# BMCV/SuperDSM

Hardware: AMD Instinct MI355X
Metric: candidate DSM solves/sec (higher is better)
Workload: dtype f64; 1 GPU; bbbc039_like 520x696 (BASELINE.json configs[1] stand-in: ellipses at the centres/areas of 8 different reference BBBC039 regression tables), 8 images per step in ONE launch, all candidates of every image: connected atom subsets of size <= 3 + cluster universes; gather_payload_bytes_per_rank=0, ranks=1, ranks_per_gpu=1, devices_visible=1, median_N=1325, median_M=23, parallelism=single GPU, steps_in_flight=1

## Files before the change

include/sdsm.h:

```cpp
#ifndef SDSM_H
#define SDSM_H

#include <stddef.h>
#include <stdint.h>

#ifdef __cplusplus
extern "C" {
#endif

#define SDSM_VERSION 200

typedef enum {
    SDSM_OK = 0,
    SDSM_ERR_ARGUMENT = -1,
    SDSM_ERR_DEVICE = -2,
    SDSM_ERR_WORKSPACE = -3,
    SDSM_ERR_UNSUPPORTED = -4
} sdsm_status;

typedef struct {
    double scale;
    double epsilon;
    double alpha;
    double smooth_amount;
// ... 61 lines not shown
size_t sdsm_plan_workspace_bytes(const sdsm_plan *plan);
size_t sdsm_plan_mask_bytes(const sdsm_plan *plan);
int sdsm_plan_describe(const sdsm_plan *plan, int32_t *mask_info, int64_t *mask_offset, int32_t *n_pixels);
int64_t sdsm_plan_total_pixels(const sdsm_plan *plan);

int sdsm_batch_upload(const sdsm_plan *plan, void *d_workspace, size_t workspace_bytes, void *stream);
int sdsm_batch_launch(const sdsm_plan *plan, const double *d_y, const int32_t *d_atoms, const uint8_t *d_valid,
                      void *d_workspace, size_t workspace_bytes, sdsm_record *d_records, uint32_t *d_masks,
                      double *d_xi, void *stream);
int sdsm_batch_launch_multi(const sdsm_plan *plan, const double *const *d_y, const int32_t *const *d_atoms, const uint8_t *const *d_valid,
                            void *d_workspace, size_t workspace_bytes, sdsm_record *d_records, uint32_t *d_masks, double *d_xi, void *stream);
int64_t sdsm_plan_xi_count(const sdsm_plan *plan);
int sdsm_plan_layout(const sdsm_plan *plan, int64_t *out);
int sdsm_plan_set_latency_mode(sdsm_plan *plan, int mode);
int sdsm_plan_schedule(const sdsm_plan *plan, int32_t *group_members, int32_t *rows_workgroups);
int sdsm_plan_xi_offsets(const sdsm_plan *plan, int64_t *xi_offset);

typedef struct {
    double contrast;
    double interior_mean;
    double exterior_mean;
    double fg_mean, fg_std;
    int32_t area;
    int32_t status;
    int32_t r0, c0, h, w;
} sdsm_post_record;
int sdsm_post_objects(const double *d_g, const double *d_gs, const uint8_t *d_bg, int H, int W, int n, const int32_t *d_boxes,
                      const int64_t *d_bits_off, const uint32_t *d_bits, const int64_t *d_new_off, uint32_t *d_new_bits,
                      uint32_t *d_boundary_pool, const int64_t *d_bpool_off, double exterior_scale, double exterior_offset,
                      double contrast_epsilon, double inv_gstd, int max_distance, double stdamp, sdsm_post_record *d_out, void *stream);
// ... 218 lines not shown
```

superdsm_amd/_capi.py:

```python
import ctypes as C
import os

import numpy as np

_HERE = os.path.dirname(os.path.abspath(__file__))
LIB_PATH = os.environ.get('SDSM_HIP_LIB', os.path.join(_HERE, 'libsdsm_hip.so'))

SDSM_OK = 0
ATOM_STATS_STRIDE = 6

CAND_OPTIMAL, CAND_FALLBACK, CAND_TRIVIAL, CAND_ERROR, CAND_UNSUPPORTED, CAND_GIVEN_UP = 0, 1, 2, 3, 4, 5


class DsmConfig(C.Structure):
    _fields_ = [('scale', C.c_double), ('epsilon', C.c_double), ('alpha', C.c_double), ('smooth_amount', C.c_double),
                ('gaussian_shape_multiplier', C.c_double), ('background_margin', C.c_double),
                ('smooth_subsample', C.c_int32), ('init_elliptical', C.c_int32), ('max_iters', C.c_int32), ('flags', C.c_int32)]


RECORD_DTYPE = np.dtype([
    ('energy', 'f8'), ('theta', 'f8', 6), ('energy_ell', 'f8'),
    ('status', 'i4'), ('flags', 'i4'), ('n_pixels', 'i4'), ('n_deform', 'i4'),
    ('iters_ell', 'i4'), ('iters_dsm', 'i4'), ('evals_value', 'i4'), ('evals_full', 'i4'),
    ('on_boundary', 'i4'), ('fg_r0', 'i4'), ('fg_c0', 'i4'), ('fg_h', 'i4'), ('fg_w', 'i4'), ('n_positive', 'i4'), ('n_negative', 'i4'), ('reserved', 'i4')])
# ... 63 lines not shown
    'sdsm_image_prepare': (_i32, [_vp, _vp, _vp, _i32, _i32, _f64, _i32, _vp, _vp, _vp, _sz, _vp]),
    'sdsm_plan_create': (_vp, [_i32, _i32, _i32, _vp, C.POINTER(DsmConfig), _i32, _vp, _vp]),
    'sdsm_plan_create_multi': (_vp, [_i32, _vp, _vp, _vp, _vp, C.POINTER(DsmConfig), _i32, _vp, _vp, _vp]),
    'sdsm_plan_destroy': (None, [_vp]),
    'sdsm_plan_workspace_bytes': (_sz, [_vp]),
    'sdsm_plan_mask_bytes': (_sz, [_vp]),
    'sdsm_plan_describe': (_i32, [_vp, _vp, _vp, _vp]),
    'sdsm_plan_total_pixels': (_i64, [_vp]),
    'sdsm_batch_upload': (_i32, [_vp, _vp, _sz, _vp]),
    'sdsm_batch_launch': (_i32, [_vp, _vp, _vp, _vp, _vp, _sz, _vp, _vp, _vp, _vp]),
    'sdsm_batch_launch_multi': (_i32, [_vp, _vp, _vp, _vp, _vp, _sz, _vp, _vp, _vp, _vp]),
    'sdsm_plan_xi_count': (_i64, [_vp]),
    'sdsm_plan_xi_offsets': (_i32, [_vp, _vp]),
    'sdsm_plan_layout': (_i32, [_vp, _vp]),
    'sdsm_plan_schedule': (_i32, [_vp, _vp, _vp]),
    'sdsm_plan_set_latency_mode': (_i32, [_vp, _i32]),
    'sdsm_post_objects': (_i32, [_vp, _vp, _vp, _i32, _i32, _i32, _vp, _vp, _vp, _vp, _vp, _vp, _vp, _f64, _f64, _f64, _f64, _i32, _f64, _vp, _vp]),
    'sdsm_post_objects_multi': (_i32, [C.POINTER(PostImage), _i32, _vp, _vp, _vp, _vp, _vp, _vp, _vp, _f64, _f64, _f64, _i32, _f64, _vp, _vp]),
    'sdsm_post_background_multi': (_i32, [C.POINTER(PostBgImage), _i32, _vp, _vp, _vp, _i32, _vp]),
    'sdsm_post_fill_holes': (_i32, [_i32, _vp, _vp, _vp, _vp, _vp, _vp, _vp, _vp]),
    'sdsm_post_glare_multi': (_i32, [C.POINTER(PostImage), _i32, _vp, _vp, _vp, C.POINTER(C.c_double), _i32, _vp, _vp, _vp, _vp]),
    'sdsm_gaussian_workspace_bytes': (_sz, [_i32, _i32, _f64]),
    'sdsm_gaussian_filter': (_i32, [_vp, _i32, _i32, _f64, _vp, _vp, _sz, _vp]),
    'sdsm_separable_workspace_bytes': (_sz, [_i32, _i32, _i32, _i32]),
    'sdsm_separable_filter': (_i32, [_vp, _i32, _i32, _vp, _i32, _vp, _i32, _vp, _vp, _sz, _vp]),
    'sdsm_log_masks_workspace_bytes': (_sz, [_i32, _i32]),
    'sdsm_log_masks': (_i32, [_vp, _i32, _i32, _i32, _vp, _vp, _vp, _vp, _sz, _vp]),
    'sdsm_integral_image': (_i32, [_vp, _i32, _i32, _vp, _vp]),
    'sdsm_doh_cube': (_i32, [_vp, _i32, _i32, _i32, _vp, _vp, _vp, _vp, _vp]),
    'sdsm_doh_peaks': (_i32, [_vp, _i32, _i32, _i32, _f64, _vp, _i64, _vp]),
# ... 103 lines not shown
```

superdsm_amd/csrc/sdsm_api.hip:

```cpp
#include <algorithm>
#include <atomic>
#include <cmath>
#include <cstdio>
#include <cstdlib>
#include <cstring>
#include <numeric>
#include <string>
#include <vector>

#include "sdsm_common.h"
#include <climits>

extern "C" hipError_t sdsm_launch_solve(const BatchParams &P, sdsm_record *records, uint32_t *masks, double *xi_out, hipStream_t stream,
                                        hipStream_t side1, hipStream_t side2, hipStream_t side3, hipStream_t side4, hipEvent_t *ev, int n_c, int n_d, int n_w, int n_r);
extern "C" hipError_t sdsm_image_prepare_impl(const double *, const uint8_t *, const int32_t *, int, int, double, int, uint8_t *, int32_t *, void *, hipStream_t);
extern "C" hipError_t sdsm_preprocess_impl(const double *, int, int, double, double, double, int, double *, void *, hipStream_t);
extern "C" void sdsm_gauss_kernel_host(double sigma, int radius, double *w);
extern "C" hipError_t sdsm_launch_setup(const BatchParams &P, hipStream_t stream, const int32_t *order_w, int n_w, int cls, const int32_t *order_small, int n_small, const int32_t *order_big, int n_big);
extern "C" int sdsm_setup_fits_small(int h, int w, int mcap, int max_label, int k);
extern "C" int sdsm_setup_class(int max_dim, int max_mcap, int max_label, int k);

static thread_local std::string g_err;
static int fail(int code, const std::string &msg) { g_err = msg; return code; }
static int hipfail(hipError_t e, const char *what) { return fail(SDSM_ERR_DEVICE, std::string(what) + ": " + hipGetErrorString(e)); }
// ... 96 lines not shown
struct sdsm_plan {
    int n = 0;
    std::vector<PlanImage> images;
    sdsm_dsm_config cfg{};
    int k = 1, R = 0, zcap = 1, zcap_run = 1, zshift = 0, no_deform = 0;
    std::vector<CandDesc> cand;
    std::vector<int32_t> fp_labels, order;
    int n_order_c = 0, n_order_d = 0, n_order_w = 0;
    int n_order_r = 0;
    int rows_mcap = 1;
    int n_setup_small = 0, n_setup_big = 0, max_label = 1;
    int setup_class = 2;
    int mode = 0;
    int wide_pixels = INT_MAX;
    int boost_pixels = INT_MAX;
    std::vector<float> psf;
    std::vector<int32_t> mask_info, n_pixels;
    std::vector<int64_t> mask_off_bytes, xi_off;
    int64_t total_pixels = 0, total_runs = 0, total_ell = 0, total_xi = 0, total_mask_words = 0, n_hglob = 0, n_wide = 0;
    size_t off_cand = 0, off_state = 0, off_fp = 0, off_order = 0, off_crop_y = 0, off_crop_rc = 0, off_crop_cc = 0, off_dist = 0, off_tmp_y = 0, off_tmp_rc = 0, off_inv = 0, off_run_meta = 0,
           off_run_q0 = 0, off_run_aux = 0, off_grid = 0, off_ell_im = 0, off_ell_w = 0, off_psf = 0, off_env_fst = 0, off_env_rb = 0, off_hglob = 0, off_wide = 0, off_ticket = 0, total = 0;
    uint64_t layout_gen = 0;
    mutable const double *x0 = nullptr;
    mutable uint64_t uploaded_gen = 0;
    mutable const void *uploaded_ws = nullptr;
    mutable SideSet *sides = nullptr;
};

#include <mutex>
static std::mutex g_pool_mutex;
static std::vector<SideSet *> g_side_sets;

static hipError_t acquire_sides(const sdsm_plan *p, hipStream_t caller)
{
    int dev = 0;
    hipError_t e = hipGetDevice(&dev);
    if (e != hipSuccess) return e;
    int sdev = dev;
    if (caller && hipStreamGetDevice(caller, &sdev) == hipSuccess && sdev != dev) return hipErrorInvalidDevice;
    (void)hipGetLastError();
    if (p->sides) return p->sides->device == dev ? hipSuccess : hipErrorInvalidDevice;
    std::lock_guard<std::mutex> lock(g_pool_mutex);
    for (SideSet *q : g_side_sets) if (q->device == dev) { p->sides = q; return hipSuccess; }
    SideSet *s = new SideSet();
    s->device = dev;
// ... 27 lines not shown
#ifndef SDSM_ROWS_MAX_REGIONS
#define SDSM_ROWS_MAX_REGIONS 1024
#endif
#ifndef SDSM_WIDE_TP_MIN_PIXELS
#define SDSM_WIDE_TP_MIN_PIXELS 8192
#endif
#ifndef SDSM_K1_PIXDIV
#define SDSM_K1_PIXDIV 2048
#endif
#ifndef SDSM_WIDE_FILL
#define SDSM_WIDE_FILL 1024
#endif
#ifndef SDSM_WIDE_MAX_MEMBERS
#define SDSM_WIDE_MAX_MEMBERS 256
#endif
static void layout_plan(sdsm_plan *p)
{
    const int n = p->n;
    const bool latency = p->mode == 1, groups = p->mode != 2;
    p->wide_pixels = latency ? SDSM_WIDE_PIXELS : INT_MAX;
    p->boost_pixels = INT_MAX;
    p->layout_gen++;
    p->n_wide = 0;
    long long wide_thr = SDSM_WIDE_MIN_PIXELS;
    if (groups && !latency) {
        long long all_pixels = 0;
        for (int i = 0; i < n; i++) all_pixels += p->cand[i].N;
        long long tp_min = SDSM_WIDE_TP_MIN_PIXELS;
        if (const char *e = getenv("SDSM_WIDE_TP_MIN_PIXELS")) { const long long v = atoll(e); if (v > 0) tp_min = v; }
        wide_thr = std::max<long long>(tp_min, all_pixels / SDSM_WIDE_FILL);
// ... 1 lines not shown
    if (!latency) {
        long long all_pixels = 0;
        for (int i = 0; i < n; i++) all_pixels += p->cand[i].N;
        long long div = SDSM_K1_PIXDIV;
        if (const char *e = getenv("SDSM_K1_PIXDIV")) { const long long v = atoll(e); if (v > 0) div = v; else if (v < 0) div = 0; }
        p->boost_pixels = div > 0 ? (int)std::min<long long>(INT_MAX, std::max<long long>(SDSM_WIDE_PIXELS, all_pixels / div)) : INT_MAX;
    }
    long wide_slice = SDSM_WIDE_SLICE;
    if (const char *e = getenv("SDSM_WIDE_SLICE")) { const long v = atol(e); if (v > 0) wide_slice = v; }
    auto group_size = [&](long N) -> long {
        if (!groups || n >= (1 << 24)) return 0;
        if (N > wide_thr) return std::min<long>(SDSM_WIDE_MAX_G, std::max<long>(2, (N + wide_slice - 1) / wide_slice));
        if (latency && N > SDSM_WIDE_PIXELS) return std::min<long>(SDSM_LAT_GMAX, std::max<long>(2, (N + SDSM_LAT_SLICE - 1) / SDSM_LAT_SLICE));
        return 0;
    };
    std::vector<char> grouped(n, 1);
    {
        std::vector<int> big;
        for (int i = 0; i < n; i++) if (group_size(p->cand[i].N) > 0) big.push_back(i);
        std::stable_sort(big.begin(), big.end(), [&](int a, int b) { return p->cand[a].N > p->cand[b].N; });
        long members = 0;
        int cutoff = 0;
        for (int i : big) {
            members += group_size(p->cand[i].N);
            if (members > SDSM_WIDE_MAX_MEMBERS) { cutoff = p->cand[i].N; break; }
        }
        for (int i : big) if (p->cand[i].N <= cutoff) grouped[i] = 0;
    }
    long rows_regions = 0;
    for (int i = 0; i < n; i++) rows_regions += p->cand[i].N > SDSM_ROWS_MIN_PIXELS;
    const bool rows_multi = rows_regions <= SDSM_ROWS_MAX_REGIONS;
    for (int i = 0; i < n; i++) {
        CandDesc &c = p->cand[i];
        const long G = grouped[i] ? group_size(c.N) : 0;
        const long RG = rows_multi && c.N > SDSM_ROWS_MIN_PIXELS && n < (1 << 24) ? std::min<long>(SDSM_ROWS_MAX_G, (c.N + SDSM_ROWS_SLICE - 1) / SDSM_ROWS_SLICE) : 0;
        c.rows_g = (int32_t)std::max<long>(RG, G > 0 ? 1 : 0);
        c.pad1 = 0;
        c.wide_g = (int32_t)G;
        if (G > 0 || c.rows_g > 0) { c.wide_off = p->n_wide; p->n_wide += SDSM_WIDE_SYNC + (int64_t)2 * G * SDSM_WIDE_PBUF; }
        else c.wide_off = -1;
    }
    p->n_order_c = p->n_order_d = p->n_order_w = p->n_order_r = 0;
    p->rows_mcap = 1;
    p->order.resize(n);
    std::iota(p->order.begin(), p->order.end(), 0);
    std::stable_sort(p->order.begin(), p->order.end(), [&](int a, int b) { return p->cand[a].N > p->cand[b].N; });
    for (int k = 0; k < n; k++) if (6 + p->cand[p->order[k]].Mcap > SDSM_K1_DENSE_N || p->cand[p->order[k]].N > SDSM_WIDE_PIXELS) { p->order.push_back(p->order[k]); p->n_order_c++; }
    for (int k = 0; k < n; k++) if (6 + p->cand[p->order[k]].Mcap > SDSM_ENV_DENSE_N) { p->order.push_back(p->order[k]); p->n_order_d++; }
    for (int k = 0; k < n; k++) {
        const int ci = p->order[k];
        for (int g = 0; g < p->cand[ci].wide_g; g++) { p->order.push_back(ci | (g << 24)); p->n_order_w++; }
    }
    for (int k = 0; k < n; k++) {
        const int ci = p->order[k];
        for (int g = 0; g < p->cand[ci].rows_g; g++) { p->order.push_back(ci | (g << 24)); p->n_order_r++; }
        if (p->cand[ci].rows_g > 0) p->rows_mcap = std::max(p->rows_mcap, (int)std::min<int64_t>(p->cand[ci].Mcap, SDSM_MAX_N_GLOBAL));
// ... 151 lines not shown
    if (mask_offset) memcpy(mask_offset, p->mask_off_bytes.data(), p->mask_off_bytes.size() * 8);
    if (n_pixels) memcpy(n_pixels, p->n_pixels.data(), p->n_pixels.size() * 4);
    return SDSM_OK;
}

extern "C" int sdsm_plan_schedule(const sdsm_plan *p, int32_t *group_members, int32_t *rows_workgroups)
{
    if (!p) return fail(SDSM_ERR_ARGUMENT, "sdsm_plan_schedule: null plan");
    for (int i = 0; i < p->n; i++) {
        if (group_members) group_members[i] = p->cand[i].wide_g;
        if (rows_workgroups) rows_workgroups[i] = p->cand[i].rows_g;
    }
    return SDSM_OK;
}

extern "C" int sdsm_plan_xi_offsets(const sdsm_plan *p, int64_t *xi_offset)
{
    if (!p || !xi_offset) return fail(SDSM_ERR_ARGUMENT, "sdsm_plan_xi_offsets: null argument");
    memcpy(xi_offset, p->xi_off.data(), p->xi_off.size() * 8);
    return SDSM_OK;
}

extern "C" int sdsm_plan_layout(const sdsm_plan *p, int64_t *out)
{
    if (!p || !out) return fail(SDSM_ERR_ARGUMENT, "sdsm_plan_layout: null argument");
    int64_t v[16] = {(int64_t)p->off_cand, (int64_t)p->off_state, (int64_t)p->off_crop_y, (int64_t)p->off_crop_rc, (int64_t)p->off_crop_cc,
                     (int64_t)p->off_run_meta, (int64_t)p->off_grid, (int64_t)p->off_ell_im, (int64_t)p->off_ell_w, p->zcap_run, p->k,
                     (int64_t)sizeof(CandDesc), p->total_pixels, p->total_ell, (int64_t)sizeof(CandState), p->total_runs};
    memcpy(out, v, sizeof(v));
    return SDSM_OK;
// ... 148 lines not shown
extern "C" int sdsm_set_debug_buffer(void *d_buf) { g_prof = (long long *)d_buf; return SDSM_OK; }


#ifndef SDSM_HESS_THR
#define SDSM_HESS_THR 0.1f
#endif
static std::atomic<int> g_solver_diag{0};
static BatchParams make_params(const sdsm_plan *p, void *d_ws)
{
    uint8_t *b = (uint8_t *)d_ws;
    BatchParams P{};
    P.n = p->n; P.n_total = p->n; P.latency = p->mode == 1; P.n_images = (int)p->images.size();
    for (size_t i = 0; i < p->images.size(); i++) { P.img[i].H = p->images[i].H; P.img[i].W = p->images[i].W; }
    P.k = p->k; P.R = p->R; P.subsample = p->cfg.smooth_subsample; P.zcap = p->zcap; P.zcap_run = p->zcap_run; P.zshift = p->zshift; P.no_deform = p->no_deform; P.no_trivial_rule = p->cfg.flags & 1;
    P.init_elliptical = p->cfg.init_elliptical; P.max_iters = p->cfg.max_iters; P.k1_pixmax = p->wide_pixels; P.boost_pixels = p->boost_pixels; P.rows_mcap = p->rows_mcap; P.pad2 = g_solver_diag.load(std::memory_order_relaxed);
    P.scale = p->cfg.scale; P.epsilon = p->cfg.epsilon; P.alpha = p->cfg.alpha; P.reg_unit = p->cfg.alpha * std::sqrt(p->cfg.epsilon);
    P.cand = (const CandDesc *)(b + p->off_cand); P.state = (CandState *)(b + p->off_state);
    P.fp_labels = (const int32_t *)(b + p->off_fp); P.order = (const int32_t *)(b + p->off_order);
    P.crop_y = (double *)(b + p->off_crop_y); P.crop_rc = (uint32_t *)(b + p->off_crop_rc); P.crop_cc = (uint32_t *)(b + p->off_crop_cc);
    P.dist = (uint32_t *)(b + p->off_dist); P.grid_rc = (uint32_t *)(b + p->off_grid);
    P.ell_im = (uint32_t *)(b + p->off_ell_im); P.ell_w = (float *)(b + p->off_ell_w); P.run_meta = (uint32_t *)(b + p->off_run_meta);
    P.run_q0 = (uint32_t *)(b + p->off_run_q0); P.run_aux = (uint32_t *)(b + p->off_run_aux);
    P.tmp_y = (double *)(b + p->off_tmp_y); P.tmp_rc = (uint32_t *)(b + p->off_tmp_rc); P.inv = (uint32_t *)(b + p->off_inv);
    P.hess_thr = SDSM_HESS_THR;
    P.psf = (const float *)(b + p->off_psf);
    P.env_fst = (int32_t *)(b + p->off_env_fst); P.env_rb = (int32_t *)(b + p->off_env_rb);
    P.hglob = (double *)(b + p->off_hglob); P.wide_pool = (double *)(b + p->off_wide);
    P.wide_ticket = (int32_t *)(b + p->off_ticket); P.wide_timeout = g_wide_timeout;
    P.cls_count = (int32_t *)(b + p->off_ticket) + 16;
    P.prof = g_prof; P.prof2 = g_prof ? g_prof + (size_t)16 * p->n : nullptr;
// ... 16 lines not shown

static double elapsed(int a, int b)
{
    if (!g_ev_valid) return -1.0;
    if (hipEventSynchronize(g_ev[b]) != hipSuccess) return -1.0;
    float ms = 0;
    if (hipEventElapsedTime(&ms, g_ev[a], g_ev[b]) != hipSuccess) return -1.0;
    return ms;
}
extern "C" double sdsm_last_setup_kernel_ms(void) { return elapsed(0, 1); }

extern "C" int sdsm_set_solver_diagnostics(int flags)
{
    if (flags & ~1) return fail(SDSM_ERR_ARGUMENT, "sdsm_set_solver_diagnostics: unknown flag bit (1: recompute at unchanged iterates)");
    g_solver_diag.store(flags, std::memory_order_relaxed);
    return SDSM_OK;
}

extern "C" int sdsm_batch_solver_counters(const sdsm_plan *p, void *d_ws, int64_t out[4])
{
    if (!p || !d_ws || !out) return fail(SDSM_ERR_ARGUMENT, "sdsm_batch_solver_counters: null argument");
    if (p->uploaded_ws != d_ws) return fail(SDSM_ERR_ARGUMENT, "sdsm_batch_solver_counters: not the workspace of the plan's upload (sdsm_batch_upload)");
    out[0] = out[1] = out[2] = out[3] = 0;
    if (p->n == 0) return SDSM_OK;
    hipError_t e;
    if ((e = hipDeviceSynchronize()) != hipSuccess) return hipfail(e, "hipDeviceSynchronize");
    if ((e = hipMemcpy(out, (const uint8_t *)d_ws + p->off_ticket + 64 + 4 * SDSM_SOLVER_COUNTERS, 8, hipMemcpyDeviceToHost)) != hipSuccess) return hipfail(e, "hipMemcpy");
    return SDSM_OK;
}
extern "C" double sdsm_last_solve_kernel_ms(void) { return elapsed(1, 2); }
// ... 784 lines not shown
```

superdsm_amd/csrc/sdsm_common.h:

```cpp
#pragma once
#include <hip/hip_runtime.h>
#include <stdint.h>
#include "../../include/sdsm.h"

#define SDSM_GLOBAL __attribute__((address_space(1)))
typedef const double SDSM_GLOBAL *g_cdouble_p;
typedef const float SDSM_GLOBAL *g_cfloat_p;
typedef const uint32_t SDSM_GLOBAL *g_cu32_p;
typedef const uint16_t SDSM_GLOBAL *g_cu16_p;
typedef float f32x4 __attribute__((ext_vector_type(4)));
typedef unsigned short u16x4 __attribute__((ext_vector_type(4)));
typedef const f32x4 SDSM_GLOBAL *g_cf32x4_p;
typedef const u16x4 SDSM_GLOBAL *g_cu16x4_p;

#define SDSM_WG 256
#define SDSM_WAVES (SDSM_WG / 64)

#define SDSM_MAX_LABELS 65535
#define SDSM_MAX_BBOX_DIM 4096
#define SDSM_PSF_LDS 4256
#define SDSM_MAX_GRID 2048
#define SDSM_K1_NMAX 128
#define SDSM_K1_EMAX 2560
#define SDSM_K1B_NMAX 256
#define SDSM_K1B_EMAX 7168
#define SDSM_K2B_NMAX 512
#define SDSM_K2B_EMAX 15170
#ifndef SDSM_WIDE_MIN_PIXELS
#define SDSM_WIDE_MIN_PIXELS 12288
#endif
#ifndef SDSM_WIDE_SLICE
#define SDSM_WIDE_SLICE 8192
#endif
#define SDSM_WIDE_MAX_G 8
#define SDSM_WIDE_SYNC 16
#define SDSM_WIDE_FCAP 4104
#define SDSM_WIDE_PBUF (SDSM_K2B_EMAX + SDSM_MAX_N_SOLVE + 64 + SDSM_WIDE_FCAP)
#define SDSM_WIDE_PIXELS 3072
#define SDSM_K2_EMAX 11000
#define SDSM_K1_DENSE_N 70
#define SDSM_ENV_DENSE_N 146
#define SDSM_RUN 4
#define SDSM_MAX_ELL_GROUPS 256
#define SDSM_HZREG 8
#define SDSM_MSLOTS 16
#define SDSM_SUPER 8
#ifndef SDSM_PANEL
#define SDSM_PANEL 4
#endif
// ... 72 lines not shown

struct BatchParams {
    int32_t n, n_images;
    int32_t n_total, latency;
    ImageRef img[SDSM_MAX_IMAGES];
    int32_t k, R, subsample, zcap;
    int32_t zcap_run, zshift;
    int32_t no_deform;
    int32_t no_trivial_rule;
    int32_t init_elliptical, max_iters;
    int32_t k1_pixmax;
    double scale, epsilon, alpha;
    double reg_unit;
    float hess_thr;
    int32_t boost_pixels;
    int32_t rows_mcap, pad2;
    const CandDesc *cand;
    CandState *state;
    const int32_t *fp_labels;
    const int32_t *order;
    double *crop_y;
    uint32_t *crop_rc;
    uint32_t *run_meta;
    uint32_t *run_q0;
    uint32_t *run_aux;
    double *tmp_y;
    uint32_t *tmp_rc;
    uint32_t *crop_cc;
    uint32_t *dist;
    uint32_t *inv;
// ... 2 lines not shown
    uint32_t *ell_im;
    int32_t *env_fst;
    int32_t *env_rb;
    const float *psf;
    double *wide_pool;
    int32_t *wide_ticket;
    long long wide_timeout;
#define SDSM_SOLVER_COUNTERS 32
    int32_t *cls_count;
    double *hglob;
    long long *prof;
    long long *prof2;
    const double *x0;
};

enum { SDSM_CLS_NONE = -1, SDSM_CLS_1 = 0, SDSM_CLS_1B = 1, SDSM_CLS_2 = 2, SDSM_CLS_2B = 3, SDSM_CLS_3 = 4, SDSM_CLS_WIDE = 5, SDSM_CLS_WIDE2B = 6 };
__host__ __device__ __forceinline__ int sdsm_solve_class(int status, int M, int env_size, int N, int wide_g, int k1_pixmax)
{
    if (status != ST_OK) return SDSM_CLS_NONE;
    int Mfull = M;
    if (6 + Mfull > SDSM_MAX_N_GLOBAL) Mfull = 0;
    const int nfull = 6 + Mfull, efull = Mfull > 0 ? env_size : 21;
    if (wide_g > 0 && nfull <= SDSM_MAX_N_SOLVE && efull <= SDSM_K2_EMAX) return SDSM_CLS_WIDE;
    if (wide_g > 0 && nfull <= SDSM_K2B_NMAX && efull <= SDSM_K2B_EMAX) return SDSM_CLS_WIDE2B;
    if (nfull <= SDSM_K1_NMAX && efull <= SDSM_K1_EMAX && N <= k1_pixmax) return SDSM_CLS_1;
    if (nfull <= SDSM_K1B_NMAX && efull <= SDSM_K1B_EMAX && N <= k1_pixmax) return SDSM_CLS_1B;
    if (nfull <= SDSM_MAX_N_SOLVE && efull <= SDSM_K2_EMAX) return SDSM_CLS_2;
    if (nfull <= SDSM_K2B_NMAX && efull <= SDSM_K2B_EMAX) return SDSM_CLS_2B;
    return SDSM_CLS_3;
}

__device__ __forceinline__ double wave_sum(double v)
{
#pragma unroll
    for (int o = 32; o > 0; o >>= 1) v += __shfl_xor(v, o);
    return v;
}
// ... 158 lines not shown
```

superdsm_amd/csrc/sdsm_solve.hip:

```cpp
#include "sdsm_common.h"
#include "sdsm_logtab.h"
#include <climits>
#include <cstdlib>
#include <type_traits>

extern __shared__ __align__(16) unsigned char sdsm_smem[];

namespace {

#define LOG_DBL_MAX 709.782712893384
#define NEWTON_ABSTOL 1e-7
#define NEWTON_RELTOL 1e-6
#define LS_ALPHA 0.01
#define LS_BETA 0.5
#define LS_K 4
#define LS_SWEEPS 10
#define LS_T0_ELL 4.0
#if defined(SDSM_PROFILE) && defined(SDSM_PROFILE_FINE)
#define FINE_FENCE() asm volatile("s_waitcnt vmcnt(0) lgkmcnt(0)" ::: "memory")
#define FINE_ADD(slot) do { FINE_FENCE(); long long _t = PROF_NOW(); prof_acc[slot] += _t - ft; ft = _t; } while (0)
#define FINE_START() long long ft = PROF_NOW()
#else
#define FINE_ADD(slot) do { } while (0)
#define FINE_START() do { } while (0)
// ... 2 lines not shown
#define EBATCH 4
#endif
#ifndef SDSM_FACTOR_DIV
#define SDSM_FACTOR_DIV 1
#ifndef SDSM_K1_THREADS
#define SDSM_K1_THREADS 192
#endif
#ifndef SDSM_K1_WPE
#define SDSM_K1_WPE 3
#endif
#ifndef SDSM_K1B_THREADS
#define SDSM_K1B_THREADS 256
#define SDSM_K1B_WPE 2
#endif
#endif
#define HZREG SDSM_HZREG
#define NSLOT SDSM_MSLOTS

template <int NMAX_, int EMAX_, bool GLOBALH = false, int WGSIZE = 256>
struct Lay {
    static constexpr int NMAX = NMAX_, EMAX = EMAX_;
    static constexpr int WGS = WGSIZE, NWAVES = WGSIZE / 64;
    static constexpr bool GLOBAL_H = GLOBALH;
    static constexpr int W = NMAX + 2;
    static constexpr int LT = 0, B0 = 2 * SDSM_LOGTAB_N;
    static constexpr int X = B0, G = B0 + W, D = B0 + 2 * W, XT = B0 + 3 * W, SC = B0 + 4 * W, YROW = B0 + 5 * W, TMP = B0 + 6 * W;
    static constexpr int RED = B0 + 7 * W, FLAG = RED + NWAVES * 32, KEPT = FLAG + 2, MS = KEPT + 4, IB = MS + 42 * NSLOT;
    static constexpr int NPANEL = NMAX / SDSM_PANEL + 2;
    static constexpr int IB_DOUBLES = (2 * W + NPANEL + 1) / 2;
    static constexpr int HP = IB + IB_DOUBLES;
    static constexpr int END = HP + (GLOBALH ? 0 : EMAX);
    static constexpr int TOTAL_BYTES = ((END * 8 + 15) / 16) * 16;
};

#define SD ((double *)sdsm_smem)

#ifdef SDSM_PROFILE
#define PROF_ARG , prof_acc
#define PROF_PARAM , long long *prof_acc
#else
#define PROF_ARG
#define PROF_PARAM
#endif

typedef double f64x2 __attribute__((ext_vector_type(2)));
typedef const f64x2 SDSM_GLOBAL *g_cf64x2_p;

struct Cand {
// ... 1111 lines not shown
            for (int cc = 0; cc < NB; cc++) {
                double acc = v[cc];
#pragma unroll
                for (int m = 0; m < cc; m++) acc -= v[m] * t[cc][m];
                v[cc] = acc * rinv[cc];
            }
#pragma unroll
            for (int cc = 0; cc < NB; cc++) if (cc < nb) row[cc] = v[cc];
        }
        PROF_ADD(11, pf);
    }
    __syncthreads();
    PROF_ADD(14, pf);
    if (failed) return failed;
    const double l2 = wave_canon_sum(n, [&](int i) { return yrow[i] * yrow[i]; });
    if (L::NMAX <= 128 || n <= 256 || (L::NMAX >= 512 && n <= 512)) {
        if (n <= 64) back_substitute_wave<1>(Hp, yrow, dg, rbp, fstp, zl, n, tid);
        else if constexpr (L::NMAX <= 128) back_substitute_wave<2>(Hp, yrow, dg, rbp, fstp, zl, n, tid);
        else if (n <= 256) back_substitute_wave<4>(Hp, yrow, dg, rbp, fstp, zl, n, tid);
        else if constexpr (L::NMAX >= 512) back_substitute_wave<8>(Hp, yrow, dg, rbp, fstp, zl, n, tid);
        __syncthreads();
    } else {
        for (int j0 = ((n - 1) / NB) * NB; j0 >= 0; j0 -= NB) {
            const int nb = n - j0 < NB ? n - j0 : NB;
            int f4[NB];
    #pragma unroll
            for (int cc = 0; cc < NB; cc++) f4[cc] = cc < nb ? uni(fstp[j0 + cc]) : j0;
            const int start = j0 + nb - 1 >= M ? 0 : f4[0];
            if (tid < NB || start + tid < j0) {
                double z[NB];
    #pragma unroll
                for (int cc = NB - 1; cc >= 0; cc--) {
                    double acc = cc < nb ? yrow[j0 + cc] : 0.0;
    #pragma unroll
                    for (int m = cc + 1; m < NB; m++) if (m < nb) acc -= Hp[rbp[j0 + m] + j0 + cc] * z[m];
// ... 172 lines not shown
    if (st.status != ST_OK) {
        if (handles_rest && tid == 0) {
            sdsm_record r = {};
            r.status = st.status == ST_TRIVIAL ? SDSM_CAND_TRIVIAL : (st.status == ST_UNSUPPORTED ? SDSM_CAND_UNSUPPORTED : SDSM_CAND_ERROR);
            r.n_pixels = cd.N;
            r.n_positive = st.npos; r.n_negative = st.nneg;
            *rec = r;
        }
        return;
    }
    int Mfull = st.M;
    bool unsupported = false;
    if (6 + Mfull > SDSM_MAX_N_GLOBAL) { unsupported = true; Mfull = 0; }
    const int efull = Mfull > 0 ? st.env_size : 21;
    {
        const int cls = sdsm_solve_class(st.status, st.M, st.env_size, cd.N, cd.wide_g, P.k1_pixmax);
        if (accept_any ? !(cls >= SDSM_CLS_1B && cls <= SDSM_CLS_3) : cls != CLS) return;
    }
    if (GLOBALH && cd.hglob_off < 0) {
        if (tid == 0) { sdsm_record r0 = {}; r0.status = SDSM_CAND_UNSUPPORTED; r0.n_pixels = cd.N; r0.n_deform = st.M; *rec = r0; }
        return;
    }

    Cand c;
    c.N = cd.N; c.NR = st.NR; c.hzmax = Mfull > 0 ? st.hzmax : 0; c.env_size = 21;
    c.p_lo = 0; c.p_hi = st.NR; c.wg = 0; c.wG = 1; c.wpool = nullptr; c.wtimeout = P.wide_timeout;
    if (WIDE) {
        c.wG = cd.wide_g; c.wg = wg; c.wpool = P.wide_pool + cd.wide_off;
        const int sup = 64 * SDSM_SUPER;
        const int chunk = (((st.NR + c.wG - 1) / c.wG) + sup - 1) / sup * sup;
        c.p_lo = wg * chunk < st.NR ? wg * chunk : st.NR;
// ... 231 lines not shown
    if constexpr (!WIDE) {
        int *sh = reinterpret_cast<int *>(SD + L::FLAG);
        for (;;) {
            __syncthreads();
            if (tid == 0) *sh = __hip_atomic_fetch_add(&P.cls_count[list], 1, __ATOMIC_RELAXED, __HIP_MEMORY_SCOPE_AGENT);
            __syncthreads();
            const int i = uni(*sh);
            if (i >= P.n) return;
            const int ci = uni(P.order[i]);
            __syncthreads();
            solve_candidate<NMAX, EMAX, GLOBALH, WGSIZE, false, CLS>(P, ci, 0, handles_rest, false, records, masks, xi_out);
        }
    }
    if constexpr (WIDE) {
        int *tk = reinterpret_cast<int *>(SD + L::FLAG);
        if (tid == 0) *tk = __hip_atomic_fetch_add(P.wide_ticket + (CLS == SDSM_CLS_WIDE2B ? 1 : 0), 1, __ATOMIC_RELAXED, __HIP_MEMORY_SCOPE_AGENT);
        __syncthreads();
        const int slot = uni(*tk);
        __syncthreads();
        if (slot >= P.n) return;
        const int entry = uni(P.order[slot]);
        solve_candidate<NMAX, EMAX, GLOBALH, WGSIZE, true, CLS>(P, entry & 0xffffff, (entry >> 24) & 0xff, handles_rest, false, records, masks, xi_out);
    }
}

template <int NMAX, int EMAX, bool GLOBALH, int WGSIZE>
__global__ __launch_bounds__(WGSIZE) void sdsm_k_eval(BatchParams P, int nprev, int eprev, const double *params, double *out)
{
    using L = Lay<NMAX, EMAX, GLOBALH, WGSIZE>;
    const int tid = threadIdx.x;
    const int ci = blockIdx.x;
// ... 180 lines not shown
                                        int n_c, int n_d, int n_w, int n_r)
{
    hipError_t e;
    BatchParams Pw = P;
    Pw.order = P.order + P.n + n_c + n_d; Pw.n = n_w;
    BatchParams Pc = P, Pd = P;
    Pc.order = P.order + P.n; Pc.n = n_c;
    Pd.order = P.order + P.n + n_c; Pd.n = n_d;
    const int g_c = n_c < SDSM_RESIDENT_2 ? n_c : SDSM_RESIDENT_2, g_d = n_d < SDSM_RESIDENT_2B ? n_d : SDSM_RESIDENT_2B, g_3 = n_d < SDSM_RESIDENT_3 ? n_d : SDSM_RESIDENT_3;
    const int g_b = n_c < SDSM_RESIDENT_1B ? n_c : SDSM_RESIDENT_1B;
    if (n_r > 0 && (e = sdsm_launch_setup_rows(P, stream, Pw.order + n_w, n_r)) != hipSuccess) return e;
    if (n_c > 0 || n_d > 0 || n_w > 0) { if ((e = hipEventRecord(ev[0], stream)) != hipSuccess) return e; }
    hipError_t first = hipSuccess;
    auto keep = [&](hipError_t r) { if (first == hipSuccess && r != hipSuccess) first = r; return first == hipSuccess; };
    bool forked1 = false, forked2 = false, forked3 = false, forked4 = false;
    const bool own_2b = sdsm_solve_wants_own_2b(n_w, n_d) && side4 != nullptr;
    if (n_d > 0 || n_w > 0) {
        if (keep(hipStreamWaitEvent(side1, ev[0], 0))) {
            forked1 = true;
            if (n_w > 0 && first == hipSuccess) keep(launch_class<SDSM_K2B_NMAX, SDSM_K2B_EMAX, 2, false, 512, true, SDSM_CLS_WIDE2B>(Pw, n_w, -1, 0, records, masks, xi_out, side1));
            if (n_d > 0 && first == hipSuccess) keep(launch_class<SDSM_MAX_N_GLOBAL, SDSM_MAX_N_GLOBAL * (SDSM_MAX_N_GLOBAL + 1) / 2, 2, true, 512, false, SDSM_CLS_3>(Pd, g_3, 3, 0, records, masks, xi_out, side1));
            if (n_d > 0 && !own_2b && first == hipSuccess) keep(launch_class<SDSM_K2B_NMAX, SDSM_K2B_EMAX, 2, false, 512, false, SDSM_CLS_2B>(Pd, g_d, 2, 0, records, masks, xi_out, side1));
        }
    }
    if (own_2b && first == hipSuccess) {
        if (keep(hipStreamWaitEvent(side4, ev[0], 0))) {
            forked4 = true;
            keep(launch_class<SDSM_K2B_NMAX, SDSM_K2B_EMAX, 2, false, 512, false, SDSM_CLS_2B>(Pd, g_d, 2, 0, records, masks, xi_out, side4));
        }
    }
    if ((n_w > 0 || n_c > 0) && first == hipSuccess) {
        if (keep(hipStreamWaitEvent(side2, ev[0], 0))) {
            forked2 = true;
            if (n_w > 0 && first == hipSuccess) keep(launch_class<SDSM_MAX_N_SOLVE, SDSM_K2_EMAX, 2, false, 512, true, SDSM_CLS_WIDE>(Pw, n_w, -1, 0, records, masks, xi_out, side2));
            if (n_c > 0 && first == hipSuccess) keep(launch_class<SDSM_MAX_N_SOLVE, SDSM_K2_EMAX, 2, false, 512, false, SDSM_CLS_2>(Pc, g_c, 1, 0, records, masks, xi_out, side2));
        }
    }
    if (n_c > 0 && first == hipSuccess) {
        if (keep(hipStreamWaitEvent(side3, ev[0], 0))) {
            forked3 = true;
            keep(launch_class<SDSM_K1B_NMAX, SDSM_K1B_EMAX, SDSM_K1B_WPE, false, SDSM_K1B_THREADS, false, SDSM_CLS_1B>(Pc, g_b, 0, 0, records, masks, xi_out, side3));
        }
    }
    if ((n_c > 0 || n_d > 0 || n_w > 0) && first == hipSuccess) {
        const int l0 = n_w > 0 ? -2 : 3, c0 = n_w > 0 ? n_w : n_d;
        const int l1 = n_w > 0 ? -1 : 1, c1 = n_w > 0 ? n_w : n_c;
        hipLaunchKernelGGL(sdsm_k_gate, dim3(1), dim3(64), 0, stream, (const int32_t *)P.cls_count, (const int32_t *)P.wide_ticket, l0, c0, l1, c1, 0, n_c,
                           (long long)SDSM_GATE_CAP_US * 100, (long long)SDSM_GATE_STALL_US * 100);
    }
    static const int resident_1 = [] { const char *e = getenv("SDSM_RESIDENT_1"); const int v = e ? atoi(e) : 0; return v > 0 ? v : SDSM_RESIDENT_1; }();
    const int g_1 = P.n < resident_1 ? P.n : resident_1;
    if (first == hipSuccess) {
        if (!P.latency) keep(launch_class<SDSM_K1_NMAX, SDSM_K1_EMAX, SDSM_K1_WPE, false, SDSM_K1_THREADS, false, SDSM_CLS_1>(P, g_1, 4, 1, records, masks, xi_out, stream));
        else keep(launch_class<SDSM_K1_NMAX, SDSM_K1_EMAX, 3, false, 256, false, SDSM_CLS_1>(P, g_1, 4, 1, records, masks, xi_out, stream));
    }
    if (forked1) { hipError_t r = hipEventRecord(ev[1], side1); if (r == hipSuccess) r = hipStreamWaitEvent(stream, ev[1], 0); keep(r); }
    if (forked2) { hipError_t r = hipEventRecord(ev[2], side2); if (r == hipSuccess) r = hipStreamWaitEvent(stream, ev[2], 0); keep(r); }
    if (forked3) { hipError_t r = hipEventRecord(ev[3], side3); if (r == hipSuccess) r = hipStreamWaitEvent(stream, ev[3], 0); keep(r); }
    if (forked4) { hipError_t r = hipEventRecord(ev[4], side4); if (r == hipSuccess) r = hipStreamWaitEvent(stream, ev[4], 0); keep(r); }
    return first;
}
// ... 1 lines not shown
```

Baseline: 682,400 candidate solves/s.

## Add light wide-group solve class with smaller LDS layout and bonus group members

Adds a new solve class for wide (multi-workgroup) candidates whose system size and envelope fit a smaller LDS layout, so a light group member can share a compute unit with a class-1 workgroup. This is meant to cut LDS-limited occupancy stalls. It also grants an extra group member to the largest wide candidates, routes the wide tickets and gate to the new class, and still launches the old wide kernel when some candidates exceed the light limits. In exchange it adds another kernel launch, more classification logic and more wide-buffer memory.

```diff
diff --git a/include/sdsm.h b/include/sdsm.h
--- a/include/sdsm.h
+++ b/include/sdsm.h
@@ -99,6 +99,8 @@
 int sdsm_plan_layout(const sdsm_plan *plan, int64_t *out);
 int sdsm_plan_set_latency_mode(sdsm_plan *plan, int mode);
 int sdsm_plan_schedule(const sdsm_plan *plan, int32_t *group_members, int32_t *rows_workgroups);
+int sdsm_plan_solve_classes(const sdsm_plan *plan, const int32_t *status, const int32_t *M, const int32_t *env_size, int32_t *cls);
+int sdsm_set_light_envelope_limit(int doubles);
 int sdsm_plan_xi_offsets(const sdsm_plan *plan, int64_t *xi_offset);
 
 typedef struct {
diff --git a/superdsm_amd/_capi.py b/superdsm_amd/_capi.py
--- a/superdsm_amd/_capi.py
+++ b/superdsm_amd/_capi.py
@@ -101,6 +101,8 @@
     'sdsm_plan_xi_offsets': (_i32, [_vp, _vp]),
     'sdsm_plan_layout': (_i32, [_vp, _vp]),
     'sdsm_plan_schedule': (_i32, [_vp, _vp, _vp]),
+    'sdsm_plan_solve_classes': (_i32, [_vp, _vp, _vp, _vp, _vp]),
+    'sdsm_set_light_envelope_limit': (_i32, [_i32]),
     'sdsm_plan_set_latency_mode': (_i32, [_vp, _i32]),
     'sdsm_post_objects': (_i32, [_vp, _vp, _vp, _i32, _i32, _i32, _vp, _vp, _vp, _vp, _vp, _vp, _vp, _f64, _f64, _f64, _f64, _i32, _f64, _vp, _vp]),
     'sdsm_post_objects_multi': (_i32, [C.POINTER(PostImage), _i32, _vp, _vp, _vp, _vp, _vp, _vp, _vp, _f64, _f64, _f64, _i32, _f64, _vp, _vp]),
diff --git a/superdsm_amd/csrc/sdsm_api.hip b/superdsm_amd/csrc/sdsm_api.hip
--- a/superdsm_amd/csrc/sdsm_api.hip
+++ b/superdsm_amd/csrc/sdsm_api.hip
@@ -134,6 +134,7 @@
     int mode = 0;
     int wide_pixels = INT_MAX;
     int boost_pixels = INT_MAX;
+    int wide_rest = 0;
     std::vector<float> psf;
     std::vector<int32_t> mask_info, n_pixels;
     std::vector<int64_t> mask_off_bytes, xi_off;
@@ -149,6 +150,7 @@
 
 #include <mutex>
 static std::mutex g_pool_mutex;
+static std::atomic<int> g_light_emax{-1};
 static std::vector<SideSet *> g_side_sets;
 
 static hipError_t acquire_sides(const sdsm_plan *p, hipStream_t caller)
@@ -206,6 +208,22 @@
 #ifndef SDSM_WIDE_MAX_MEMBERS
 #define SDSM_WIDE_MAX_MEMBERS 256
 #endif
+#ifndef SDSM_WIDE_BONUS
+#define SDSM_WIDE_BONUS 1
+#endif
+#ifndef SDSM_WIDE_BONUS_PCT
+#define SDSM_WIDE_BONUS_PCT 90
+#endif
+#ifndef SDSM_LIGHT_MIN_CANDIDATES
+#define SDSM_LIGHT_MIN_CANDIDATES 1024
+#endif
+static int light_limit(const sdsm_plan *p)
+{
+    if (!SDSM_LIGHT_GROUPS || p->n_order_w <= 0) return 0;
+    const int v = g_light_emax.load(std::memory_order_relaxed);
+    if (v >= 0) return v;
+    return p->n > SDSM_LIGHT_MIN_CANDIDATES ? SDSM_KL_EMAX : 0;
+}
 static void layout_plan(sdsm_plan *p)
 {
     const int n = p->n;
@@ -237,7 +255,7 @@
         if (latency && N > SDSM_WIDE_PIXELS) return std::min<long>(SDSM_LAT_GMAX, std::max<long>(2, (N + SDSM_LAT_SLICE - 1) / SDSM_LAT_SLICE));
         return 0;
     };
-    std::vector<char> grouped(n, 1);
+    std::vector<char> grouped(n, 1), bonus(n, 0);
     {
         std::vector<int> big;
         for (int i = 0; i < n; i++) if (group_size(p->cand[i].N) > 0) big.push_back(i);
@@ -249,13 +267,23 @@
             if (members > SDSM_WIDE_MAX_MEMBERS) { cutoff = p->cand[i].N; break; }
         }
         for (int i : big) if (p->cand[i].N <= cutoff) grouped[i] = 0;
+        if (SDSM_WIDE_BONUS > 0 && groups && !latency) {
+            long used = 0, nmax = 0;
+            for (int i : big) if (grouped[i]) { used += group_size(p->cand[i].N); nmax = std::max<long>(nmax, p->cand[i].N); }
+            for (int i : big) {
+                if (!grouped[i] || 6 + (long)p->cand[i].Mcap <= SDSM_KL_NMAX || (long long)p->cand[i].N * 100 < (long long)nmax * SDSM_WIDE_BONUS_PCT) continue;
+                const long g = group_size(p->cand[i].N);
+                const long b = std::min<long>(std::min<long>(SDSM_WIDE_BONUS, SDSM_WIDE_MAX_G - g), SDSM_WIDE_MAX_MEMBERS - used);
+                if (b > 0) { bonus[i] = (char)b; used += b; }
+            }
+        }
     }
     long rows_regions = 0;
     for (int i = 0; i < n; i++) rows_regions += p->cand[i].N > SDSM_ROWS_MIN_PIXELS;
     const bool rows_multi = rows_regions <= SDSM_ROWS_MAX_REGIONS;
     for (int i = 0; i < n; i++) {
         CandDesc &c = p->cand[i];
-        const long G = grouped[i] ? group_size(c.N) : 0;
+        const long G = grouped[i] ? group_size(c.N) + bonus[i] : 0;
         const long RG = rows_multi && c.N > SDSM_ROWS_MIN_PIXELS && n < (1 << 24) ? std::min<long>(SDSM_ROWS_MAX_G, (c.N + SDSM_ROWS_SLICE - 1) / SDSM_ROWS_SLICE) : 0;
         c.rows_g = (int32_t)std::max<long>(RG, G > 0 ? 1 : 0);
         c.pad1 = 0;
@@ -263,6 +291,8 @@
         if (G > 0 || c.rows_g > 0) { c.wide_off = p->n_wide; p->n_wide += SDSM_WIDE_SYNC + (int64_t)2 * G * SDSM_WIDE_PBUF; }
         else c.wide_off = -1;
     }
+    p->wide_rest = 0;
+    for (int i = 0; i < n; i++) if (p->cand[i].wide_g > 0 && 6 + (long)p->cand[i].Mcap > SDSM_K2B_NMAX) p->wide_rest = 1;
     p->n_order_c = p->n_order_d = p->n_order_w = p->n_order_r = 0;
     p->rows_mcap = 1;
     p->order.resize(n);
@@ -444,6 +474,14 @@
     return SDSM_OK;
 }
 
+extern "C" int sdsm_plan_solve_classes(const sdsm_plan *p, const int32_t *status, const int32_t *M, const int32_t *env_size, int32_t *cls)
+{
+    if (!p || !status || !M || !env_size || !cls) return fail(SDSM_ERR_ARGUMENT, "sdsm_plan_solve_classes: null argument");
+    const int light = light_limit(p);
+    for (int i = 0; i < p->n; i++) cls[i] = sdsm_solve_class(status[i], M[i], env_size[i], p->cand[i].N, p->cand[i].wide_g, p->wide_pixels, light);
+    return SDSM_OK;
+}
+
 extern "C" int sdsm_plan_xi_offsets(const sdsm_plan *p, int64_t *xi_offset)
 {
     if (!p || !xi_offset) return fail(SDSM_ERR_ARGUMENT, "sdsm_plan_xi_offsets: null argument");
@@ -622,6 +660,7 @@
     for (size_t i = 0; i < p->images.size(); i++) { P.img[i].H = p->images[i].H; P.img[i].W = p->images[i].W; }
     P.k = p->k; P.R = p->R; P.subsample = p->cfg.smooth_subsample; P.zcap = p->zcap; P.zcap_run = p->zcap_run; P.zshift = p->zshift; P.no_deform = p->no_deform; P.no_trivial_rule = p->cfg.flags & 1;
     P.init_elliptical = p->cfg.init_elliptical; P.max_iters = p->cfg.max_iters; P.k1_pixmax = p->wide_pixels; P.boost_pixels = p->boost_pixels; P.rows_mcap = p->rows_mcap; P.pad2 = g_solver_diag.load(std::memory_order_relaxed);
+    P.light_emax = light_limit(p); P.pad3 = p->wide_rest;
     P.scale = p->cfg.scale; P.epsilon = p->cfg.epsilon; P.alpha = p->cfg.alpha; P.reg_unit = p->cfg.alpha * std::sqrt(p->cfg.epsilon);
     P.cand = (const CandDesc *)(b + p->off_cand); P.state = (CandState *)(b + p->off_state);
     P.fp_labels = (const int32_t *)(b + p->off_fp); P.order = (const int32_t *)(b + p->off_order);
@@ -668,6 +707,13 @@
 {
     if (flags & ~1) return fail(SDSM_ERR_ARGUMENT, "sdsm_set_solver_diagnostics: unknown flag bit (1: recompute at unchanged iterates)");
     g_solver_diag.store(flags, std::memory_order_relaxed);
+    return SDSM_OK;
+}
+
+extern "C" int sdsm_set_light_envelope_limit(int doubles)
+{
+    if (doubles > SDSM_KL_EMAX) return fail(SDSM_ERR_ARGUMENT, "sdsm_set_light_envelope_limit: at most SDSM_KL_EMAX (12400) doubles fit the light layout");
+    g_light_emax.store(doubles < 0 ? -1 : doubles, std::memory_order_relaxed);
     return SDSM_OK;
 }
 
diff --git a/superdsm_amd/csrc/sdsm_common.h b/superdsm_amd/csrc/sdsm_common.h
--- a/superdsm_amd/csrc/sdsm_common.h
+++ b/superdsm_amd/csrc/sdsm_common.h
@@ -33,6 +33,11 @@
 #define SDSM_WIDE_SLICE 8192
 #endif
 #define SDSM_WIDE_MAX_G 8
+#define SDSM_KL_NMAX 288
+#define SDSM_KL_EMAX 12400
+#ifndef SDSM_LIGHT_GROUPS
+#define SDSM_LIGHT_GROUPS 1
+#endif
 #define SDSM_WIDE_SYNC 16
 #define SDSM_WIDE_FCAP 4104
 #define SDSM_WIDE_PBUF (SDSM_K2B_EMAX + SDSM_MAX_N_SOLVE + 64 + SDSM_WIDE_FCAP)
@@ -135,6 +140,7 @@
     double reg_unit;
     float hess_thr;
     int32_t boost_pixels;
+    int32_t light_emax, pad3;
     int32_t rows_mcap, pad2;
     const CandDesc *cand;
     CandState *state;
@@ -167,13 +173,17 @@
     const double *x0;
 };
 
-enum { SDSM_CLS_NONE = -1, SDSM_CLS_1 = 0, SDSM_CLS_1B = 1, SDSM_CLS_2 = 2, SDSM_CLS_2B = 3, SDSM_CLS_3 = 4, SDSM_CLS_WIDE = 5, SDSM_CLS_WIDE2B = 6 };
-__host__ __device__ __forceinline__ int sdsm_solve_class(int status, int M, int env_size, int N, int wide_g, int k1_pixmax)
+enum { SDSM_CLS_NONE = -1, SDSM_CLS_1 = 0, SDSM_CLS_1B = 1, SDSM_CLS_2 = 2, SDSM_CLS_2B = 3, SDSM_CLS_3 = 4, SDSM_CLS_WIDE = 5, SDSM_CLS_WIDE2B = 6, SDSM_CLS_WIDE_LIGHT = 7 };
+__host__ __device__ __forceinline__ int sdsm_solve_class(int status, int M, int env_size, int N, int wide_g, int k1_pixmax, int light_emax)
 {
     if (status != ST_OK) return SDSM_CLS_NONE;
     int Mfull = M;
     if (6 + Mfull > SDSM_MAX_N_GLOBAL) Mfull = 0;
     const int nfull = 6 + Mfull, efull = Mfull > 0 ? env_size : 21;
+    if (wide_g > 0 && light_emax > 0) {
+        if (nfull <= SDSM_KL_NMAX && efull <= light_emax) return SDSM_CLS_WIDE_LIGHT;
+        if (nfull <= SDSM_K2B_NMAX && efull <= SDSM_K2B_EMAX) return SDSM_CLS_WIDE2B;
+    }
     if (wide_g > 0 && nfull <= SDSM_MAX_N_SOLVE && efull <= SDSM_K2_EMAX) return SDSM_CLS_WIDE;
     if (wide_g > 0 && nfull <= SDSM_K2B_NMAX && efull <= SDSM_K2B_EMAX) return SDSM_CLS_WIDE2B;
     if (nfull <= SDSM_K1_NMAX && efull <= SDSM_K1_EMAX && N <= k1_pixmax) return SDSM_CLS_1;
diff --git a/superdsm_amd/csrc/sdsm_solve.hip b/superdsm_amd/csrc/sdsm_solve.hip
--- a/superdsm_amd/csrc/sdsm_solve.hip
+++ b/superdsm_amd/csrc/sdsm_solve.hip
@@ -40,6 +40,10 @@
 #define SDSM_K1B_WPE 2
 #endif
 #endif
+#ifndef SDSM_KL_THREADS
+#define SDSM_KL_THREADS 512
+#endif
+#define SDSM_KL_WPE (SDSM_KL_THREADS == 512 ? 3 : 2)
 #define HZREG SDSM_HZREG
 #define NSLOT SDSM_MSLOTS
 
@@ -58,6 +62,12 @@
     static constexpr int END = HP + (GLOBALH ? 0 : EMAX);
     static constexpr int TOTAL_BYTES = ((END * 8 + 15) / 16) * 16;
 };
+
+constexpr int lds_granules(int bytes, int granule) { return (bytes + granule - 1) / granule; }
+#define SDSM_LIGHT_FITS(K1T, GRAN) (lds_granules(Lay<SDSM_KL_NMAX, SDSM_KL_EMAX, false, SDSM_KL_THREADS>::TOTAL_BYTES, GRAN) + lds_granules(Lay<SDSM_K1_NMAX, SDSM_K1_EMAX, false, K1T>::TOTAL_BYTES, GRAN) <= 160 * 1024 / (GRAN))
+static_assert(Lay<SDSM_KL_NMAX, SDSM_KL_EMAX, false, SDSM_KL_THREADS>::TOTAL_BYTES <= 126576 && Lay<SDSM_K1_NMAX, SDSM_K1_EMAX, false, SDSM_K1_THREADS>::TOTAL_BYTES <= 36432, "light group layout: 126 576 bytes beside class 1's 36 176 (36 432 at 256 threads)");
+static_assert(SDSM_LIGHT_FITS(SDSM_K1_THREADS, 1280) && SDSM_LIGHT_FITS(256, 1280) && SDSM_LIGHT_FITS(SDSM_K1_THREADS, 512) && SDSM_LIGHT_FITS(256, 512), "a light group member and one class-1 workgroup share the 160 KB of a compute unit");
+static_assert(SDSM_KL_EMAX + SDSM_KL_NMAX <= SDSM_K2B_EMAX + SDSM_MAX_N_SOLVE && SDSM_KL_NMAX <= SDSM_K2B_NMAX && SDSM_KL_EMAX <= SDSM_K2B_EMAX, "SDSM_WIDE_PBUF is sized by the largest group layout; every light group fits the layout of class 2b");
 
 #define SD ((double *)sdsm_smem)
 
@@ -1199,11 +1209,11 @@
     PROF_ADD(14, pf);
     if (failed) return failed;
     const double l2 = wave_canon_sum(n, [&](int i) { return yrow[i] * yrow[i]; });
-    if (L::NMAX <= 128 || n <= 256 || (L::NMAX >= 512 && n <= 512)) {
+    if (L::NMAX <= 128 || n <= 256 || (L::NMAX > 256 && n <= 512)) {
         if (n <= 64) back_substitute_wave<1>(Hp, yrow, dg, rbp, fstp, zl, n, tid);
         else if constexpr (L::NMAX <= 128) back_substitute_wave<2>(Hp, yrow, dg, rbp, fstp, zl, n, tid);
         else if (n <= 256) back_substitute_wave<4>(Hp, yrow, dg, rbp, fstp, zl, n, tid);
-        else if constexpr (L::NMAX >= 512) back_substitute_wave<8>(Hp, yrow, dg, rbp, fstp, zl, n, tid);
+        else if constexpr (L::NMAX > 256) back_substitute_wave<(L::NMAX < 512 ? (L::NMAX + 63) / 64 : 8)>(Hp, yrow, dg, rbp, fstp, zl, n, tid);
         __syncthreads();
     } else {
         for (int j0 = ((n - 1) / NB) * NB; j0 >= 0; j0 -= NB) {
@@ -1406,7 +1416,7 @@
     if (6 + Mfull > SDSM_MAX_N_GLOBAL) { unsupported = true; Mfull = 0; }
     const int efull = Mfull > 0 ? st.env_size : 21;
     {
-        const int cls = sdsm_solve_class(st.status, st.M, st.env_size, cd.N, cd.wide_g, P.k1_pixmax);
+        const int cls = sdsm_solve_class(st.status, st.M, st.env_size, cd.N, cd.wide_g, P.k1_pixmax, P.light_emax);
         if (accept_any ? !(cls >= SDSM_CLS_1B && cls <= SDSM_CLS_3) : cls != CLS) return;
     }
     if (GLOBALH && cd.hglob_off < 0) {
@@ -1668,7 +1678,7 @@
     }
     if constexpr (WIDE) {
         int *tk = reinterpret_cast<int *>(SD + L::FLAG);
-        if (tid == 0) *tk = __hip_atomic_fetch_add(P.wide_ticket + (CLS == SDSM_CLS_WIDE2B ? 1 : 0), 1, __ATOMIC_RELAXED, __HIP_MEMORY_SCOPE_AGENT);
+        if (tid == 0) *tk = __hip_atomic_fetch_add(P.wide_ticket + (CLS == SDSM_CLS_WIDE_LIGHT ? 2 : CLS == SDSM_CLS_WIDE2B ? 1 : 0), 1, __ATOMIC_RELAXED, __HIP_MEMORY_SCOPE_AGENT);
         __syncthreads();
         const int slot = uni(*tk);
         __syncthreads();
@@ -1879,6 +1889,7 @@
     hipError_t first = hipSuccess;
     auto keep = [&](hipError_t r) { if (first == hipSuccess && r != hipSuccess) first = r; return first == hipSuccess; };
     bool forked1 = false, forked2 = false, forked3 = false, forked4 = false;
+    const bool light = SDSM_LIGHT_GROUPS && P.light_emax > 0;
     const bool own_2b = sdsm_solve_wants_own_2b(n_w, n_d) && side4 != nullptr;
     if (n_d > 0 || n_w > 0) {
         if (keep(hipStreamWaitEvent(side1, ev[0], 0))) {
@@ -1897,7 +1908,8 @@
     if ((n_w > 0 || n_c > 0) && first == hipSuccess) {
         if (keep(hipStreamWaitEvent(side2, ev[0], 0))) {
             forked2 = true;
-            if (n_w > 0 && first == hipSuccess) keep(launch_class<SDSM_MAX_N_SOLVE, SDSM_K2_EMAX, 2, false, 512, true, SDSM_CLS_WIDE>(Pw, n_w, -1, 0, records, masks, xi_out, side2));
+            if (n_w > 0 && light && first == hipSuccess) keep(launch_class<SDSM_KL_NMAX, SDSM_KL_EMAX, SDSM_KL_WPE, false, SDSM_KL_THREADS, true, SDSM_CLS_WIDE_LIGHT>(Pw, n_w, -1, 0, records, masks, xi_out, side2));
+            if (n_w > 0 && (!light || P.pad3) && first == hipSuccess) keep(launch_class<SDSM_MAX_N_SOLVE, SDSM_K2_EMAX, 2, false, 512, true, SDSM_CLS_WIDE>(Pw, n_w, -1, 0, records, masks, xi_out, side2));
             if (n_c > 0 && first == hipSuccess) keep(launch_class<SDSM_MAX_N_SOLVE, SDSM_K2_EMAX, 2, false, 512, false, SDSM_CLS_2>(Pc, g_c, 1, 0, records, masks, xi_out, side2));
         }
     }
@@ -1909,7 +1921,7 @@
     }
     if ((n_c > 0 || n_d > 0 || n_w > 0) && first == hipSuccess) {
         const int l0 = n_w > 0 ? -2 : 3, c0 = n_w > 0 ? n_w : n_d;
-        const int l1 = n_w > 0 ? -1 : 1, c1 = n_w > 0 ? n_w : n_c;
+        const int l1 = n_w > 0 ? (light ? -3 : -1) : 1, c1 = n_w > 0 ? n_w : n_c;
         hipLaunchKernelGGL(sdsm_k_gate, dim3(1), dim3(64), 0, stream, (const int32_t *)P.cls_count, (const int32_t *)P.wide_ticket, l0, c0, l1, c1, 0, n_c,
                            (long long)SDSM_GATE_CAP_US * 100, (long long)SDSM_GATE_STALL_US * 100);
     }
```

After: 704,800 candidate solves/s, median of 6. +3.3%, better.
